# evergreen-ci/evergreen

Measured on NVIDIA H100. Metric: tasks scheduled/sec over N distros; host-allocator decisions/sec at 1/2/4/8 GPU, higher is better.
Workload: dtype int64

## Files before the change

### evergreen_b200/csrc/evg_plan_general.cuh

```cuda
#pragma once

#ifndef EVG_OCC_GLINK
#define EVG_OCC_GLINK 4
#endif
#ifndef EVG_OCC_GALLOC
#define EVG_OCC_GALLOC 4
#endif
#ifndef EVG_OCC_GFILL
#define EVG_OCC_GFILL 4
#endif
#ifndef EVG_OCC_GUNIT
#define EVG_OCC_GUNIT 4
#endif
#ifndef EVG_OCC_GBEST
#define EVG_OCC_GBEST 4
#endif
#ifndef EVG_GTASK_OCC
#define EVG_GTASK_OCC 2
#endif
constexpr int kGTile = 2048;

struct DGen {
  int64_t n_tiles;
  int64_t tile0;
// ... 65 lines not shown
}

__global__ void __launch_bounds__(256) k_gmark(DTasks T, DDistros D, DWork W, DGen G) {
  if (*W.err) return;
  const int tile = int(blockIdx.x + G.tile0);
  const int d = G.tile_distro[tile];
  const int64_t base = D.task_off[d], end = D.task_off[d + 1];
  const int64_t lo = max(G.tile_start[tile], base), hi = min(G.tile_start[tile] + kGTile, end);
  for (int64_t t = lo + threadIdx.x; t < hi; t += 256)
    for (int64_t e = T.dep_off[t]; e < T.dep_off[t + 1]; e++) W.has_dep[base + T.dep_idx[e]] = 1;
}

struct TileFold {
  unsigned int c[10];
  unsigned long long s[4];
  unsigned long long vmax, vmin;
};

__global__ void __launch_bounds__(256, EVG_GTASK_OCC) k_gtask(DTasks T, DDistros D, DWork W, DGen G, int64_t now, int any_complex) {
  if (*W.err) return;
  __shared__ TileFold F;
  __shared__ evg_distro_cfg s_cfg;
  __shared__ uint32_t s_nd[kNdTable];
  const int tile = int(blockIdx.x + G.tile0);
  const int d = G.tile_distro[tile];
  const int tid = threadIdx.x, lane = tid & 31;
  const unsigned full = 0xffffffffu;
  if (tid == 0) {
    for (int k = 0; k < 10; k++) F.c[k] = 0;
    for (int k = 0; k < 4; k++) F.s[k] = 0;
    F.vmax = 0ull; F.vmin = ~0ull;
    s_cfg = D.cfg[d];
  }
  __syncthreads();
  const evg_distro_cfg& cfg = s_cfg;
  const int64_t base = D.task_off[d], end = D.task_off[d + 1];
  const int64_t ts = G.tile_start[tile];
  const uint32_t ng = uint32_t(D.group_off[d + 1] - D.group_off[d]);
  const uint32_t ub = uint32_t(D.unit_base[d]);
  const bool gv = cfg.group_versions != 0;
  const int64_t threshold = cfg.target_time_ns;
  const PlannerFactors pf = clamp_factors(cfg);
  const Factors32 f32 = factors32(pf, now);
  const bool sane_clock = threshold >= 0 && now >= threshold;
  const int64_t wait_cutoff = wsub(now, threshold);
  const bool fast_clock = now >= 0 && pf.nd_int != 0;
  const bool incl = cfg.includes_dependencies != 0;
  if (tid < kNdTable) {
    const int64_t e = nd_table_entry(pf, tid);
    s_nd[tid] = (e >= 0 && e < int64_t(kNdTermLimit)) ? uint32_t(e) : 0xFFFFFFFFu;
  }
  __syncthreads();
  const bool dcomplex = any_complex && (ng > 0 || gv || (T.n_edges > 0 && T.dep_off[end] > T.dep_off[base]));

  unsigned int c_dm = 0, c_mq = 0, c_over = 0, c_wait = 0, c_sec = 0, c_ung = 0, c_ucnt = 0, c_uover = 0, c_uwait = 0, c_umq = 0;
  int64_t s_exp = 0, s_over = 0, s_uexp = 0, s_uover = 0;
  unsigned long long kmax = 0ull, kmin = ~0ull;

#pragma unroll 1
  for (int u = 0; u < 2; u++) {
    const int64_t t4 = ts + 4 * int64_t(u * 256 + tid);
    const bool live = t4 < end;
    int4 prio4 = make_int4(0, 0, 0, 0), nd4 = prio4, gid4 = make_int4(-1, -1, -1, -1), tgo4 = prio4, vid4 = prio4;
    uint4 fl4 = make_uint4(0, 0, 0, 0);
    uint32_t cmask = 0, womask = 0;
    if (live && dcomplex) {
      tgo4 = *reinterpret_cast<const int4*>(T.tgo + t4);
      if (gv) vid4 = *reinterpret_cast<const int4*>(T.vid + t4);
    }
    longlong2 ex01 = make_longlong2(0, 0), ex23 = ex01, qb01 = ex01, qb23 = ex01, wb01 = ex01, wb23 = ex01;
    if (live) {
      prio4 = *reinterpret_cast<const int4*>(T.priority + t4);
      nd4 = *reinterpret_cast<const int4*>(T.numdep + t4);
      gid4 = *reinterpret_cast<const int4*>(T.gid + t4);
      fl4 = *reinterpret_cast<const uint4*>(T.flags + t4);
      ex01 = *reinterpret_cast<const longlong2*>(T.expected + t4); ex23 = *reinterpret_cast<const longlong2*>(T.expected + t4 + 2);
      qb01 = *reinterpret_cast<const longlong2*>(T.qbasis + t4); qb23 = *reinterpret_cast<const longlong2*>(T.qbasis + t4 + 2);
      wb01 = *reinterpret_cast<const longlong2*>(T.wbasis + t4); wb23 = *reinterpret_cast<const longlong2*>(T.wbasis + t4 + 2);
    }
    int64_t doff[5] = {0, 0, 0, 0, 0};
    uint32_t hd4 = 0;
    if (live && dcomplex) {
      if (T.n_edges > 0) {
        const longlong2 d01 = *reinterpret_cast<const longlong2*>(T.dep_off + t4), d23 = *reinterpret_cast<const longlong2*>(T.dep_off + t4 + 2);
        doff[0] = d01.x; doff[1] = d01.y; doff[2] = d23.x; doff[3] = d23.y; doff[4] = T.dep_off[t4 + 4];
      }
      hd4 = *reinterpret_cast<const uint32_t*>(W.has_dep + t4);
    }
    const int32_t prio_[4] = {prio4.x, prio4.y, prio4.z, prio4.w}, nd_[4] = {nd4.x, nd4.y, nd4.z, nd4.w};
    const int32_t gid_[4] = {gid4.x, gid4.y, gid4.z, gid4.w};
    const uint32_t fl_[4] = {fl4.x, fl4.y, fl4.z, fl4.w};
    const int64_t ex_[4] = {ex01.x, ex01.y, ex23.x, ex23.y}, qb_[4] = {qb01.x, qb01.y, qb23.x, qb23.y};
    const int64_t wb_[4] = {wb01.x, wb01.y, wb23.x, wb23.y};
    int64_t vout[4];
    uint32_t eout[4], nd_term[4];
    bool wr_v[4], solo[4];
    bool dom = true;
#pragma unroll
    for (int m = 0; m < 4; m++) {
      const int64_t t = t4 + m;
      const bool valid = live & (t >= base) & (t < end);
      const int32_t prio = prio_[m], nd = nd_[m], gid = gid_[m];
      const uint32_t fl = fl_[m];
      const int64_t exp_ns = ex_[m], qb = qb_[m], wb = wb_[m];
      const bool dm = valid & ((fl & EVG_TF_DEPS_MET) != 0);
      const bool counted = valid & (!incl | dm);
      const bool over = counted & (exp_ns > threshold);
      const bool waited = sane_clock ? (wb < wait_cutoff) : (since(now, wb) > threshold);
      const bool wait_over = counted & dm & waited;
      const bool mq_dm = dm & ((fl & EVG_TF_REQ_MASK) == EVG_TF_REQ_MERGE_QUEUE);
      const bool ung = valid & (gid < 0);
      c_dm += dm; c_mq += mq_dm; c_over += over; c_wait += wait_over; c_sec += valid & ((fl & EVG_TF_OTHER_DISTRO) != 0);
      s_exp += counted ? exp_ns : 0;
      s_over += over ? exp_ns : 0;
      c_ung += ung; c_ucnt += ung & counted; c_uover += ung & over; c_uwait += ung & wait_over; c_umq += ung & mq_dm;
      s_uexp += (ung & counted) ? exp_ns : 0;
      s_uover += (ung & over) ? exp_ns : 0;
      const bool own_complex = valid & dcomplex & ((gid >= 0) | gv | (((hd4 >> (8 * m)) & 0xFFu) != 0));
      const bool complex_task = own_complex | (valid & dcomplex & (doff[m + 1] > doff[m]));
      const bool scores = valid & !own_complex;
      const uint32_t ndc = uint32_t(nd > 0 ? nd : 0);
      const uint32_t tab = s_nd[ndc < uint32_t(kNdTable) ? ndc : 0u];
      const uint32_t mul = (f32.ok & (ndc < kTask32Limit)) ? f32.nd * ndc : 0xFFFFFFFFu;
      nd_term[m] = ndc < uint32_t(kNdTable) ? tab : mul;
      dom = dom & (!scores | (score32_bad(now, prio, exp_ns, qb, nd_term[m]) == 0u));
      wr_v[m] = scores;
      solo[m] = scores & !complex_task;
      eout[m] = (valid & !complex_task) ? 1u : 0u;
      cmask |= (complex_task ? 1u : 0u) << m;
      womask |= (wait_over ? 1u : 0u) << m;
    }
    if (f32.ok_base && __all_sync(full, dom)) {
#pragma unroll
      for (int m = 0; m < 4; m++) vout[m] = int64_t(single_task_value32_nd(f32, now, prio_[m], ex_[m], qb_[m], nd_term[m], fl_[m]));
    } else {
#pragma unroll
      for (int m = 0; m < 4; m++) vout[m] = int64_t(score_slow(pf, fast_clock, wr_v[m], now, prio_[m], ex_[m], qb_[m], nd_[m], fl_[m]));
    }
#pragma unroll
    for (int m = 0; m < 4; m++) {
      const unsigned long long k = ord_i64(vout[m]);
      kmax = solo[m] ? max(kmax, k) : kmax;
      kmin = solo[m] ? min(kmin, k) : kmin;
    }
    if (!live) {
    } else if (t4 >= base && t4 + 3 < end) {
      *reinterpret_cast<longlong2*>(G.tv + t4) = make_longlong2(vout[0], vout[1]);
      *reinterpret_cast<longlong2*>(G.tv + t4 + 2) = make_longlong2(vout[2], vout[3]);
    } else {
#pragma unroll
      for (int m = 0; m < 4; m++)
        if (wr_v[m]) G.tv[t4 + m] = vout[m];
    }
    if (dcomplex && live) {
      if (t4 >= base && t4 + 3 < end) *reinterpret_cast<uint4*>(G.e + t4) = make_uint4(eout[0], eout[1], eout[2], eout[3]);
      else {
#pragma unroll
        for (int m = 0; m < 4; m++)
          if (t4 + m >= base && t4 + m < end) G.e[t4 + m] = eout[m];
      }
    }
    if (dcomplex) {
      __shared__ uint32_t s_wsum[8];
      __shared__ uint32_t s_lbase;
      const uint32_t mine = __popc(cmask);
      uint32_t inc = mine;
#pragma unroll
      for (int o = 1; o < 32; o <<= 1) { const uint32_t x = __shfl_up_sync(full, inc, o); if (lane >= o) inc += x; }
      if (lane == 31) s_wsum[tid >> 5] = inc;
      __syncthreads();
      uint32_t before = 0, total = 0;
#pragma unroll
      for (int w = 0; w < 8; w++) { const uint32_t x = s_wsum[w]; before += w < (tid >> 5) ? x : 0u; total += x; }
      if (total) {
        if (tid == 0) s_lbase = atomicAdd(G.ccount, total);
        __syncthreads();
        uint32_t pos = s_lbase + before + inc - mine;
        const int32_t vid_[4] = {vid4.x, vid4.y, vid4.z, vid4.w}, tgo_[4] = {tgo4.x, tgo4.y, tgo4.z, tgo4.w};
#pragma unroll
        for (int m = 0; m < 4; m++) {
          if (!((cmask >> m) & 1u)) continue;
          const uint32_t t = uint32_t(t4 + m), li = uint32_t(t4 + m - base);
          const int32_t gid = gid_[m], vid = vid_[m];
          const bool own_complex = (gid >= 0) | gv | (((hd4 >> (8 * m)) & 0xFFu) != 0);
          const uint32_t s_own = own_complex ? ub + own_slot_local(gid, vid, li, ng, gv) : kInactive;
          const uint32_t s_ver = (gid >= 0 && gv) ? ub + ng + uint32_t(vid) : kInactive;
          G.wl[pos] = make_uint4(t, uint32_t(d), s_own, s_ver);
          URec r;
          r.prio = prio_[m]; r.nd = nd_[m]; r.exp_ns = ex_[m]; r.qb = qb_[m]; r.tgo = tgo_[m];
          r.lif = li | (gid >= 0 ? kRecGrouped : 0u) | (((womask >> m) & 1u) ? kRecWaitOver : 0u) | ((fl_[m] & 0x3Fu) << 24);
          rec_store(G.pay + pos, r);
          pos++;
        }
      }
      __syncthreads();
    }
  }
  {
    unsigned int cs[10] = {c_dm, c_mq, c_over, c_wait, c_sec, c_ung, c_ucnt, c_uover, c_uwait, c_umq};
#pragma unroll
    for (int k = 0; k < 10; k++) cs[k] = __reduce_add_sync(full, cs[k]);
    int64_t ss[4] = {s_exp, s_over, s_uexp, s_uover};
#pragma unroll
    for (int k = 0; k < 4; k++) ss[k] = warp_sum64(ss[k]);
#pragma unroll
    for (int o = 16; o > 0; o >>= 1) {
      kmax = max(kmax, __shfl_xor_sync(full, kmax, o));
      kmin = min(kmin, __shfl_xor_sync(full, kmin, o));
    }
    if (lane == 0) {
#pragma unroll
      for (int k = 0; k < 10; k++) if (cs[k]) atomicAdd(&F.c[k], cs[k]);
#pragma unroll
      for (int k = 0; k < 4; k++) if (ss[k]) atomicAdd(&F.s[k], (unsigned long long)ss[k]);
      atomicMax(&F.vmax, kmax); atomicMin(&F.vmin, kmin);
    }
  }
  __syncthreads();
  if (tid < 16) {
    evg_queue_info* q = W.qinfo + d;
    switch (tid) {
      case 0: atomic_add64(&q->length_with_dependencies_met, F.c[0]); break;
      case 1: atomic_add64(&q->count_dep_filled_merge_queue_tasks, F.c[1]); break;
      case 2: atomic_add64(&q->count_duration_over_threshold, F.c[2]); break;
      case 3: atomic_add64(&q->count_wait_over_threshold, F.c[3]); break;
      case 4: atomic_add64(&q->secondary_queue, F.c[4]); break;
      case 5: atomic_add64(&q->has_ungrouped, F.c[5]); break;
      case 6: atomic_add64(&q->ungrouped.count, F.c[6]); break;
      case 7: atomic_add64(&q->ungrouped.count_duration_over_threshold, F.c[7]); break;
      case 8: atomic_add64(&q->ungrouped.count_wait_over_threshold, F.c[8]); break;
      case 9: atomic_add64(&q->ungrouped.count_dep_filled_merge_queue_tasks, F.c[9]); break;
      case 10: atomic_add64(&q->expected_duration, int64_t(F.s[0])); break;
      case 11: atomic_add64(&q->duration_over_threshold, int64_t(F.s[1])); break;
      case 12: atomic_add64(&q->ungrouped.expected_duration, int64_t(F.s[2])); break;
      case 13: atomic_add64(&q->ungrouped.duration_over_threshold, int64_t(F.s[3])); break;
      case 14: if (F.vmax > __ldcg(G.vmm + 2 * d)) atomicMax(G.vmm + 2 * d, F.vmax); break;
      case 15: if (F.vmin < __ldcg(G.vmm + 2 * d + 1)) atomicMin(G.vmm + 2 * d + 1, F.vmin); break;
    }
  }
}


struct WlTask {
  uint32_t t; int d; int64_t base; uint32_t li; bool own_complex; uint32_t s_own, s_ver;
};
__device__ __forceinline__ WlTask wl_task(const DDistros& D, const DGen& G, unsigned int k) {
  const uint4 e = G.wl[k];
  WlTask x;
  x.t = e.x; x.d = int(e.y); x.s_own = e.z; x.s_ver = e.w;
  x.base = D.task_off[x.d];
  x.li = uint32_t(int64_t(x.t) - x.base);
  x.own_complex = x.s_own != kInactive;
  return x;
}
template <typename F>
__device__ __forceinline__ void wl_pairs(const DTasks& T, const DGen& G, const WlTask& x, unsigned int k, F&& f) {
  if (x.own_complex) f(G.pown + k, x.s_own, true);
  if (x.s_ver != kInactive) f(G.pver + k, x.s_ver, false);
  if (T.n_edges > 0)
    for (int64_t e = T.dep_off[x.t]; e < T.dep_off[x.t + 1]; e++) {
      const uint32_t sl = G.sedge[e];
      if (sl != kInactive) f(G.pedge + e, sl, false);
    }
}

__global__ void __launch_bounds__(256, EVG_OCC_GLINK) k_glink(DTasks T, DDistros D, DWork W, DGen G, int64_t now) {
  if (*W.err) return;
  const unsigned int n = *G.ccount;
  for (unsigned int k = blockIdx.x * blockDim.x + threadIdx.x; k < n; k += gridDim.x * blockDim.x) {
    const WlTask x = wl_task(D, G, k);
    const uint32_t t = x.t;
    const int d = x.d;
    const uint32_t ub = uint32_t(D.unit_base[d]), ng = uint32_t(D.group_off[d + 1] - D.group_off[d]);
    if (x.own_complex && x.s_own - ub < ng) {
      const URec me = rec_load(G.pay + k);
      const evg_distro_cfg* cf = D.cfg + d;
      const uint32_t fl = (me.lif >> 24) & 0x3Fu;
      const int64_t exp_ns = me.exp_ns, threshold = cf->target_time_ns;
      const bool dm = (fl & EVG_TF_DEPS_MET) != 0;
      const bool counted = !cf->includes_dependencies || dm;
      const bool over = counted && exp_ns > threshold;
      const bool wait_over = (me.lif & kRecWaitOver) != 0;
      const bool mq_dm = dm && (fl & EVG_TF_REQ_MASK) == EVG_TF_REQ_MERGE_QUEUE;
      evg_group_info* g = W.ginfo + D.group_off[d] + (x.s_own - ub);
      atomic_add64(&g->count, counted);
      atomic_add64(&g->expected_duration, counted ? exp_ns : 0);
      atomic_add64(&g->count_duration_over_threshold, over);
      atomic_add64(&g->duration_over_threshold, over ? exp_ns : 0);
      atomic_add64(&g->count_wait_over_threshold, wait_over);
      atomic_add64(&g->count_dep_filled_merge_queue_tasks, mq_dm);
    }
    if (x.own_complex) G.pown[k] = atomicAdd(W.unit_n + x.s_own, 1u);
    if (x.s_ver != kInactive) G.pver[k] = atomicAdd(W.unit_n + x.s_ver, 1u);
    if (T.n_edges > 0) {
      const bool gv = D.cfg[d].group_versions != 0;
      const int64_t e0 = T.dep_off[t], e1 = T.dep_off[t + 1];
      for (int64_t e = e0; e < e1; e++) {
        const uint32_t dl = uint32_t(T.dep_idx[e]);
        const uint32_t sl = ub + own_slot_local(T.gid[x.base + dl], T.vid[x.base + dl], dl, ng, gv);
        bool dup = (sl == x.s_own) || (sl == x.s_ver);
        for (int64_t f = e0; f < e && !dup; f++) {
          const uint32_t fl2 = uint32_t(T.dep_idx[f]);
          dup = ub + own_slot_local(T.gid[x.base + fl2], T.vid[x.base + fl2], fl2, ng, gv) == sl;
        }
        G.sedge[e] = dup ? kInactive : sl;
        if (!dup) G.pedge[e] = atomicAdd(W.unit_n + sl, 1u);
      }
// ... 329 lines not shown
    } else {
#pragma unroll
      for (int m = 0; m < 8; m++) { const int64_t t = t8 + m; if (t >= base && t < end) G.e[t] = ps[m]; }
    }
    __syncthreads();
    const uint32_t total = s_total;
    const bool staged = total <= uint32_t(kStage);
#pragma unroll
    for (int m = 0; m < 8; m++) {
      const int64_t t = t8 + m;
      if (t >= base && t < end && !((dsp >> m) & 1u)) {
        if (staged) {
          const unsigned long long key = vmax_ord - ord_i64(vv[m]);
          const uint32_t q = ps[m] - p_tile;
          st_lo[q] = uint32_t(key); st_ix[q] = uint32_t(t - base);
          if (wide) st_hi[q] = uint32_t(key >> 32);
        } else {
          gen_put(G, base, ps[m], vmax_ord, wide, vv[m], uint32_t(t - base));
        }
      }
    }
    if (staged) {
      __syncthreads();
      uint32_t* dlo = G.key_lo[0] + base + p_tile;
      uint32_t* dix = G.idx[0] + base + p_tile;
      uint32_t* dhi = G.key_hi[0] + base + p_tile;
      for (uint32_t q = tid; q < total; q += 256) {
        dlo[q] = st_lo[q]; dix[q] = st_ix[q];
        if (wide) dhi[q] = st_hi[q];
      }
    }
  } else if (interior) {
    uint32_t kl[8], kh[8];
#pragma unroll
    for (int m = 0; m < 8; m++) {
      const unsigned long long key = vmax_ord - ord_i64(vv[m]);
      kl[m] = uint32_t(key); kh[m] = uint32_t(key >> 32);
    }
    const uint32_t p0 = uint32_t(t8 - base);
    *reinterpret_cast<uint4*>(G.key_lo[0] + t8) = make_uint4(kl[0], kl[1], kl[2], kl[3]);
    *reinterpret_cast<uint4*>(G.key_lo[0] + t8 + 4) = make_uint4(kl[4], kl[5], kl[6], kl[7]);
    *reinterpret_cast<uint4*>(G.idx[0] + t8) = make_uint4(p0, p0 + 1, p0 + 2, p0 + 3);
    *reinterpret_cast<uint4*>(G.idx[0] + t8 + 4) = make_uint4(p0 + 4, p0 + 5, p0 + 6, p0 + 7);
    if (wide) {
      *reinterpret_cast<uint4*>(G.key_hi[0] + t8) = make_uint4(kh[0], kh[1], kh[2], kh[3]);
      *reinterpret_cast<uint4*>(G.key_hi[0] + t8 + 4) = make_uint4(kh[4], kh[5], kh[6], kh[7]);
    }
  } else {
#pragma unroll
    for (int m = 0; m < 8; m++) {
      const int64_t t = t8 + m;
      if (t >= base && t < end) gen_put(G, base, uint32_t(t - base), vmax_ord, wide, vv[m], uint32_t(t - base));
    }
  }
}

__global__ void __launch_bounds__(256) k_gplace_disp(DTasks T, DDistros D, DWork W, DGen G) {
  const unsigned int n = *G.ccount;
  for (unsigned int k = blockIdx.x * blockDim.x + threadIdx.x; k < n; k += gridDim.x * blockDim.x) {
  const uint4 ent = G.wl[k];
  const uint32_t t = ent.x;
  if (!(W.has_dep[t] & 2)) continue;
  const int d = int(ent.y);
  const int64_t base = D.task_off[d];
  const uint4 tie = G.tie[k];
  const uint32_t a = tie.x, myrk = tie.y, slot = tie.z;
  uint32_t pos = G.e[base + a];
  const uint32_t cnt = W.unit_n[slot];
  if (cnt <= 64) {
    pos += __popcll(W.unit_mask[slot] & ((1ull << myrk) - 1ull));
  } else {
    const uint32_t* run = G.run + W.head[slot];
    for (uint32_t i = 0; i < cnt; i++) {
      const uint4 tq = G.tie[run[i] & kRunEntry];
      if (tq.z == slot && tq.y < myrk) pos++;
    }
  }
  gen_put(G, base, pos, G.vmm[2 * d], gen_bits(G, d) > 32, G.tv[t], uint32_t(int64_t(t) - base));
  }
}

__device__ __forceinline__ bool gen_tile(const DDistros& D, const DGen& G, int tile, int j, int* d_out, int64_t* seg, int64_t* lo,
                                         int* cnt, bool* wide) {
  const int d = G.tile_distro[tile];
  const int bits = gen_bits(G, d);
  if (j >= gen_npass(bits)) return false;
  const int64_t base = D.task_off[d], end = D.task_off[d + 1];
  const int64_t a = max(G.tile_start[tile], base), b = min(G.tile_start[tile] + kGTile, end);
  *d_out = d; *seg = base; *lo = a; *cnt = int(b - a); *wide = bits > 32;
  return true;
}

__global__ void __launch_bounds__(256) k_ghist(int j, DDistros D, DGen G) {
  if (j >= *G.maxpass) return;
  int d, cnt; int64_t seg, lo; bool wide;
  const int tile = int(blockIdx.x + G.tile0);
  if (!gen_tile(D, G, tile, j, &d, &seg, &lo, &cnt, &wide)) return;
  const uint32_t* src = (j < 4 ? G.key_lo[j & 1] : G.key_hi[j & 1]) + lo;
  const int shift = 8 * (j & 3);
  __shared__ uint32_t h[256];
  h[threadIdx.x] = 0;
  __syncthreads();
  for (int i = threadIdx.x; i < cnt; i += 256) atomicAdd(&h[(src[i] >> shift) & 255u], 1u);
  __syncthreads();
  G.tile_hist[int64_t(tile) * 256 + threadIdx.x] = h[threadIdx.x];
}

__global__ void __launch_bounds__(1024) k_gdscan(int j, const int32_t* __restrict__ general_list, DGen G) {
  if (j >= *G.maxpass) return;
  const int d = general_list[blockIdx.x];
  if (j >= gen_npass(gen_bits(G, d))) return;
  const int dg = threadIdx.x & 255, grp = threadIdx.x >> 8;
  const int64_t t0 = G.dtile_off[d], nt = G.dtile_off[d + 1] - t0;
  const int64_t per = (nt + 3) / 4;
  const int64_t a = t0 + (grp * per < nt ? grp * per : nt), b = t0 + ((grp + 1) * per < nt ? (grp + 1) * per : nt);
  uint32_t* h = G.tile_hist + dg;
  uint32_t sum = 0;
  int64_t tile = a;
  for (; tile + 8 <= b; tile += 8) {
    uint32_t x[8];
#pragma unroll
    for (int k = 0; k < 8; k++) x[k] = h[(tile + k) * 256];
#pragma unroll
    for (int k = 0; k < 8; k++) sum += x[k];
  }
  for (; tile < b; tile++) sum += h[tile * 256];
  __shared__ uint32_t part[4][256];
  __shared__ uint32_t s[256];
  part[grp][dg] = sum;
  __syncthreads();
  const uint32_t total = part[0][dg] + part[1][dg] + part[2][dg] + part[3][dg];
  if (grp == 0) s[dg] = total;
  __syncthreads();
  for (int o = 1; o < 256; o <<= 1) {
    uint32_t v = 0;
    if (grp == 0 && dg >= o) v = s[dg - o];
    __syncthreads();
    if (grp == 0) s[dg] += v;
    __syncthreads();
  }
  uint32_t run = s[dg] - total;
  for (int g = 0; g < grp; g++) run += part[g][dg];
  tile = a;
  for (; tile + 8 <= b; tile += 8) {
    uint32_t x[8];
#pragma unroll
    for (int k = 0; k < 8; k++) x[k] = h[(tile + k) * 256];
#pragma unroll
    for (int k = 0; k < 8; k++) { h[(tile + k) * 256] = run; run += x[k]; }
  }
  for (; tile < b; tile++) { const uint32_t x = h[tile * 256]; h[tile * 256] = run; run += x; }
}

template <bool WIDE>
__device__ __forceinline__ void gscatter_tile(int j, const DGen& G, int tile, int64_t seg, int64_t lo, int cnt, uint32_t (*wcnt)[256],
                                              uint32_t* s_lo, uint32_t* s_ix, uint32_t* s_hi, int32_t* s_delta, uint32_t* s_wsum) {
  constexpr bool wide = WIDE;
  const int sb = j & 1, db = sb ^ 1;
  const int tid = threadIdx.x, warp = tid >> 5, lane = tid & 31;
#pragma unroll
  for (int w = 0; w < 8; w++) wcnt[w][tid] = 0u;
  __syncthreads();
  const unsigned lt = (1u << lane) - 1u;
  const int shift = 8 * (j & 3);
  const bool use_hi = j >= 4;
  const uint32_t* src_lo = G.key_lo[sb] + lo;
  const uint32_t* src_hi = G.key_hi[sb] + lo;
  const uint32_t* src_ix = G.idx[sb] + lo;
  uint32_t kl[8], kh[8], ix[8], dg[8], rk[8];
#pragma unroll
  for (int k = 0; k < 8; k++) {
    const int i = (warp * 8 + k) * 32 + lane;
    const bool ok = i < cnt;
    kl[k] = ok ? src_lo[i] : 0u;
    kh[k] = (ok && wide) ? src_hi[i] : 0u;
    ix[k] = ok ? src_ix[i] : 0u;
  }
  unsigned peers[8];
#pragma unroll
  for (int k = 0; k < 8; k++) {
    const int i = (warp * 8 + k) * 32 + lane;
    dg[k] = i < cnt ? (((use_hi ? kh[k] : kl[k]) >> shift) & 255u) : 256u;
    peers[k] = __match_any_sync(0xffffffffu, dg[k]);
  }
#pragma unroll
  for (int k = 0; k < 8; k++) {
    rk[k] = 0;
    if (dg[k] < 256u && (peers[k] & lt) == 0u) rk[k] = atomicAdd(&wcnt[warp][dg[k]], uint32_t(__popc(peers[k])));
  }
#pragma unroll
  for (int k = 0; k < 8; k++) rk[k] = __shfl_sync(0xffffffffu, rk[k], __ffs(peers[k]) - 1) + uint32_t(__popc(peers[k] & lt));
  __syncthreads();
  {
    uint32_t x[8], tot = 0;
#pragma unroll
    for (int w = 0; w < 8; w++) { x[w] = wcnt[w][tid]; tot += x[w]; }
    uint32_t inc = tot;
#pragma unroll
    for (int o = 1; o < 32; o <<= 1) { const uint32_t y = __shfl_up_sync(0xffffffffu, inc, o); if (lane >= o) inc += y; }
    if (lane == 31) s_wsum[warp] = inc;
    __syncthreads();
    uint32_t before = 0;
#pragma unroll
    for (int w = 0; w < 8; w++) before += w < warp ? s_wsum[w] : 0u;
    const uint32_t lbase = before + inc - tot;
    s_delta[tid] = int32_t(G.tile_hist[int64_t(tile) * 256 + tid]) - int32_t(lbase);
    uint32_t run = lbase;
#pragma unroll
    for (int w = 0; w < 8; w++) { wcnt[w][tid] = run; run += x[w]; }
  }
  __syncthreads();
#pragma unroll
  for (int k = 0; k < 8; k++) {
    if (dg[k] < 256u) {
      const uint32_t lp = wcnt[warp][dg[k]] + rk[k];
      s_lo[lp] = kl[k];
      s_ix[lp] = ix[k];
      if (wide) s_hi[lp] = kh[k];
    }
  }
  __syncthreads();
  uint32_t* dst_lo = G.key_lo[db] + seg;
  uint32_t* dst_hi = G.key_hi[db] + seg;
  uint32_t* dst_ix = G.idx[db] + seg;
  for (int i = tid; i < cnt; i += 256) {
    const uint32_t a = s_lo[i], h = wide ? s_hi[i] : 0u;
    const uint32_t dgt = ((use_hi ? h : a) >> shift) & 255u;
    const int64_t pos = int64_t(s_delta[dgt]) + i;
    dst_lo[pos] = a;
    dst_ix[pos] = s_ix[i];
    if (wide) dst_hi[pos] = h;
  }
}

__global__ void __launch_bounds__(256, 4) k_gscatter(int j, DDistros D, DGen G) {
  if (j >= *G.maxpass) return;
  int d, cnt; int64_t seg, lo; bool wide;
  const int tile = int(blockIdx.x + G.tile0);
  if (!gen_tile(D, G, tile, j, &d, &seg, &lo, &cnt, &wide)) return;
  __shared__ uint32_t wcnt[8][256];
  __shared__ uint32_t s_lo[kGTile], s_ix[kGTile], s_hi[kGTile];
  __shared__ int32_t s_delta[256];
  __shared__ uint32_t s_wsum[8];
  if (wide) gscatter_tile<true>(j, G, tile, seg, lo, cnt, wcnt, s_lo, s_ix, s_hi, s_delta, s_wsum);
  else gscatter_tile<false>(j, G, tile, seg, lo, cnt, wcnt, s_lo, s_ix, s_hi, s_delta, s_wsum);
}

__global__ void __launch_bounds__(256) k_gemit(DDistros D, DGen G, int32_t* __restrict__ order, int64_t* __restrict__ total_value) {
  const int tile = int(blockIdx.x + G.tile0);
  const int d = G.tile_distro[tile];
  const int64_t base = D.task_off[d], end = D.task_off[d + 1];
  const int64_t lo = max(G.tile_start[tile], base), hi = min(G.tile_start[tile] + kGTile, end);
  const int bits = gen_bits(G, d);
  const int fin = gen_npass(bits) & 1;
  const bool wide = bits > 32;
  const unsigned long long vmax_ord = G.vmm[2 * d];
  for (int64_t p = lo + threadIdx.x; p < hi; p += 256) {
    unsigned long long key = G.key_lo[fin][p];
    if (wide) key |= (unsigned long long)G.key_hi[fin][p] << 32;
    order[p] = int32_t(G.idx[fin][p]);
    total_value[p] = unord_i64(vmax_ord - key);
  }
}
```

### evergreen_b200/csrc/evg_sched.cu

```cuda
#include <cuda_runtime.h>
#include <stdarg.h>
#include <stdint.h>
#include <stdio.h>
#include <string.h>

#include <algorithm>
#include <type_traits>
#include <cstdlib>
#include <future>
#include <mutex>
#include <string>
#include <vector>

#include "evg_score.cuh"
#include "evg_intern.h"

using namespace evg;

namespace {

thread_local std::string g_err;

int fail(int code, const char* fmt, ...) {
  char buf[512];
// ... 1423 lines not shown
  w.best_pair = c->b_bestpair.as<uint32_t>();
  w.buf[0].key_v = c->b_kv.as<uint64_t>();
  w.qinfo = c->b_qinfo.as<evg_queue_info>(); w.ginfo = c->b_ginfo.as<evg_group_info>();
  return w;
}
DGen dgen(const evg_ctx* c) {
  DGen g;
  g.n_tiles = c->NT;
  g.tile0 = 0;
  g.tile_distro = c->b_tiledistro.as<int32_t>(); g.tile_start = c->b_tilestart.as<int64_t>();
  g.dtile_off = c->b_dtileoff.as<int64_t>();
  g.vmm = c->b_vmm.as<unsigned long long>();
  for (int k = 0; k < 2; k++) {
    g.key_lo[k] = c->b_klo[k].as<uint32_t>(); g.key_hi[k] = c->b_khi[k].as<uint32_t>(); g.idx[k] = c->b_ix[k].as<uint32_t>();
  }
  g.e = c->b_e.as<uint32_t>(); g.tile_sum = c->b_tilesum.as<uint32_t>(); g.tile_hist = c->b_tilehist.as<uint32_t>();
  g.wl = c->b_wl.as<uint4>();
  g.pay = c->b_pay.as<URec>();
  g.pown = c->b_place.as<uint32_t>();
  g.pver = c->b_place.as<uint32_t>() + (c->Tgc + 1);
  g.pedge = c->b_eplace.as<uint32_t>();
  g.sedge = c->b_eplace.as<uint32_t>() + (c->E + 1);
  g.ccount = c->b_gmisc.as<unsigned int>();
  g.maxpass = c->b_gmisc.as<int32_t>() + 1;
  g.rcount = c->b_gmisc.as<unsigned int>() + 2;
  g.hcount = c->b_gmisc.as<unsigned int>() + 3;
  g.bcount = c->b_gmisc.as<unsigned int>() + 4;
  g.blist = c->b_blist.as<uint2>();
  g.rank = c->b_rank.as<uint32_t>();
  g.hlist = c->b_hlist.as<uint2>();
  g.usum = c->b_usum.as<uint4>();
  g.run = c->b_run.as<uint32_t>();
  g.tie = c->b_tie.as<uint4>();
  g.tv = c->b_tv.as<int64_t>();
  return g;
}

#define LOCK(c) std::lock_guard<std::recursive_mutex> lock_((c)->mu)
#define LAUNCH_ON(c, st, kernel, grid, block, ...)                           \
  do {                                                                       \
    if ((grid) > 0) {                                                        \
      kernel<<<(grid), (block), 0, (st)>>>(__VA_ARGS__);                     \
      (c)->launches++;                                                       \
    }                                                                        \
  } while (0)
#define LAUNCH(c, kernel, grid, block, ...) LAUNCH_ON(c, (c)->stream, kernel, grid, block, __VA_ARGS__)

int run_alloc_range(evg_ctx* c, int64_t now, int32_t d0, int32_t d1) {
  DHosts h;
  h.n = c->H; h.flags = c->b_hflags.as<uint32_t>(); h.gid = c->b_hgid.as<int32_t>();
  h.expected = c->b_hexp.as<int64_t>(); h.stddev = c->b_hstd.as<int64_t>(); h.start = c->b_hstart.as<int64_t>();
  h.host_off = c->b_hostoff.as<int64_t>(); h.cfg = c->b_acfg.as<evg_alloc_cfg>();
  if (c->ext_result && c->ext_capacity < c->Dn) return fail(EVG_ERR_INVALID, "bound result buffer holds %lld rows, need %d", (long long)c->ext_capacity, c->Dn);
  CK(c->b_gs.ensure(sizeof(GroupScratch) * size_t(c->G + 1)));
  const int split = (d1 - d0) >= 4096 ? 1 : 0;
  const bool listed = split && c->alist_valid && d0 == 0 && d1 == c->Dn;
  const int32_t* al = listed ? c->b_alist.as<int32_t>() : nullptr;
  const int64_t teams = listed ? c->n_alist : int64_t(d1 - d0);
  if (c->max_groups > kWideAllocGroups)
    LAUNCH(c, k_alloc<128>, unsigned(teams), 128, h, d0, d1, c->b_groupoff.as<int64_t>(), c->b_qinfo.as<evg_queue_info>(),
           c->b_ginfo.as<evg_group_info>(), c->b_gs.as<GroupScratch>(), now, c->result_ptr(), c->b_status.as<int32_t>(), split, al, int32_t(c->n_alist));
  else
    LAUNCH(c, k_alloc<32>, grid_for(teams, 4), 128, h, d0, d1, c->b_groupoff.as<int64_t>(), c->b_qinfo.as<evg_queue_info>(),
           c->b_ginfo.as<evg_group_info>(), c->b_gs.as<GroupScratch>(), now, c->result_ptr(), c->b_status.as<int32_t>(), split, al, int32_t(c->n_alist));
  if (split)
    LAUNCH(c, k_alloc_groupless, grid_for(d1 - d0, 128), 128, h, d0, d1, c->b_groupoff.as<int64_t>(), c->b_qinfo.as<evg_queue_info>(), now,
           c->result_ptr(), c->b_status.as<int32_t>());
  CK(cudaGetLastError());
  return EVG_OK;
}
int run_alloc(evg_ctx* c, int64_t now) { return run_alloc_range(c, now, 0, c->Dn); }

template <int THREADS, int ITEMS, int MIN_CTAS>
int launch_smem(evg_ctx* c, cudaStream_t st, const DTasks& dt, const DDistros& dd, const DWork& w, const int32_t* list, int32_t n,
                int64_t now, int lists_needed = 0, const int32_t* list_count = nullptr) {
  if (n <= 0) return EVG_OK;
  const size_t bytes = PlanSmem<THREADS, ITEMS>::kBytes;
  CK(cudaFuncSetAttribute(k_plan_smem<THREADS, ITEMS, MIN_CTAS>, cudaFuncAttributeMaxDynamicSharedMemorySize, int(bytes)));
  k_plan_smem<THREADS, ITEMS, MIN_CTAS><<<unsigned(n), THREADS, bytes, st>>>(dt, dd, w, list, list_count, now, lists_needed,
                                                                          c->b_order.as<int32_t>(), c->b_tv.as<int64_t>());
  c->launches++;
  return EVG_OK;
}

template <int THREADS, int CAP, int OCC>
int launch_cta(evg_ctx* c, cudaStream_t st, const DTasks& dt, const DDistros& dd, const DWork& w, const int32_t* list, int32_t n,
               int64_t now, int32_t* punt_list, int32_t* punt_count) {
  if (n <= 0) return EVG_OK;
  const size_t bytes = PlanCta<THREADS, CAP>::kBytes;
  CK(cudaFuncSetAttribute(k_plan_cta<THREADS, CAP, OCC>, cudaFuncAttributeMaxDynamicSharedMemorySize, int(bytes)));
  k_plan_cta<THREADS, CAP, OCC><<<unsigned(n), THREADS, bytes, st>>>(dt, dd, w, list, now, c->t_pad, c->b_order.as<int32_t>(),
                                                                  c->b_tv.as<int64_t>(), punt_list, punt_count);
  c->launches++;
  return EVG_OK;
}

int launch_tiny(evg_ctx* c, cudaStream_t st, const DTasks& dt, const DDistros& dd, const DWork& w, const int32_t* list, int32_t n,
                int64_t now, int lists_needed) {
  if (n <= 0) return EVG_OK;
  if (lists_needed) return launch_smem<128, 8, 8>(c, st, dt, dd, w, list, n, now, 1);
  k_plan_warp<<<grid_for(int64_t(n) * 32, 256), 256, 0, st>>>(dt, dd, w, list, n, now, c->b_order.as<int32_t>(), c->b_tv.as<int64_t>());
  c->launches++;
  return EVG_OK;
}

int prepare_general(evg_ctx* c, cudaStream_t s, int32_t d0, int32_t d1) {
  const int64_t t0 = c->h_taskoff[d0], t1 = c->h_taskoff[d1], u0 = c->h_unitbase[d0], u1 = c->h_unitbase[d1];
  const int64_t g0 = c->h_groupoff[d0], g1 = c->h_groupoff[d1], e0 = c->h_edgeoff[d0], e1 = c->h_edgeoff[d1];
  CK(cudaMemsetAsync(c->b_qinfo.as<evg_queue_info>() + d0, 0, sizeof(evg_queue_info) * size_t(d1 - d0), s));
  if (g1 > g0) CK(cudaMemsetAsync(c->b_ginfo.as<evg_group_info>() + g0, 0, sizeof(evg_group_info) * size_t(g1 - g0), s));
  if (c->general_complex) {
    const size_t nt = size_t(t1 - t0);
    CK(cudaMemsetAsync(c->b_hasdep.as<uint8_t>() + t0, 0, nt, s));
    CK(cudaMemsetAsync(c->b_unitn.as<uint32_t>() + u0, 0, sizeof(uint32_t) * size_t(u1 - u0), s));
  }
  return EVG_OK;
}

int run_general(evg_ctx* c, cudaStream_t st, const DTasks& dt, const DDistros& dd, const DWork& w, int64_t now, int32_t gfirst,
                int32_t gcount) {
  if (gcount <= 0) return EVG_OK;
  DGen g = dgen(c);
  const int gc = c->general_complex;
  const std::vector<int32_t>& gh = c->routes[kGeneral].h;
  const int32_t d_first = gh[size_t(gfirst)], d_last = gh[size_t(gfirst + gcount - 1)];
  g.tile0 = c->h_dtileoff[size_t(d_first)];
  const unsigned nt = unsigned(c->h_dtileoff[size_t(d_last) + 1] - g.tile0);
  const int32_t* gl = c->routes[kGeneral].b.as<int32_t>() + gfirst;
  LAUNCH_ON(c, st, k_ginit, grid_for(gcount, 256), 256, g, gl, gcount);
  if (gc && c->E > 0) LAUNCH_ON(c, st, k_gmark, nt, 256, dt, dd, w, g);
  if (c->timed) CK(cudaEventRecord(c->ev_gt0, st));
  LAUNCH_ON(c, st, k_gtask, nt, 256, dt, dd, w, g, now, gc);
  if (c->timed) { CK(cudaEventRecord(c->ev_gt1, st)); c->general_timed = true; }
  const unsigned wl_grid = unsigned(std::min<int64_t>(std::max<int64_t>(1, (c->Tgc + 255) / 256), int64_t(c->num_sms) * 16));
  if (gc) {
    LAUNCH_ON(c, st, k_glink, wl_grid, 256, dt, dd, w, g, now);
    LAUNCH_ON(c, st, k_galloc, wl_grid, 256, dt, dd, w, g);
    LAUNCH_ON(c, st, k_gfill, wl_grid, 256, dt, dd, w, g);
    LAUNCH_ON(c, st, k_gunit, wl_grid, 256, dd, w, g, now);
    LAUNCH_ON(c, st, k_grank, wl_grid, 256, w, g);
    LAUNCH_ON(c, st, k_gbest, wl_grid, 256, dt, dd, w, g, c->bd_valid ? 1 : 0);
  }
  LAUNCH_ON(c, st, k_gsched, grid_for(gcount, 128), 128, g, gl, gcount);
  if (gc) {
    LAUNCH_ON(c, st, k_gsum, nt, 256, dd, g);
    LAUNCH_ON(c, st, k_gscan, unsigned(gcount), 1024, g, gl);
  }
  LAUNCH_ON(c, st, k_gplace, nt, 256, dd, w, g, gc);
  if (gc) LAUNCH_ON(c, st, k_gplace_disp, wl_grid, 256, dt, dd, w, g);
  if (c->timed) CK(cudaEventRecord(c->ev_sort0, st));
  for (int j = 0; j < 8; j++) {
    LAUNCH_ON(c, st, k_ghist, nt, 256, j, dd, g);
    LAUNCH_ON(c, st, k_gdscan, unsigned(gcount), 1024, j, gl, g);
    LAUNCH_ON(c, st, k_gscatter, nt, 256, j, dd, g);
  }
  if (c->timed) CK(cudaEventRecord(c->ev_sort1, st));
  LAUNCH_ON(c, st, k_gemit, nt, 256, dd, g, c->b_order.as<int32_t>(), c->b_tv.as<int64_t>());
  const int64_t g0 = c->h_groupoff[size_t(d_first)], g1 = c->h_groupoff[size_t(d_last) + 1];
  LAUNCH_ON(c, st, k_finalize_info, grid_for(std::max<int64_t>(d_last + 1 - d_first, g1 - g0), 256), 256, dd, w, d_first, d_last + 1, g0, g1);
  return EVG_OK;
}

int ensure_aux_streams(evg_ctx* c) {
  if (c->ev_fork) return EVG_OK;
  for (int k = 0; k < evg_ctx::kAux; k++) {
    CK(cudaStreamCreateWithFlags(&c->s_aux[k], cudaStreamNonBlocking));
    CK(cudaEventCreateWithFlags(&c->ev_join[k], cudaEventDisableTiming));
  }
  CK(cudaEventCreateWithFlags(&c->ev_fork, cudaEventDisableTiming));
  return EVG_OK;
}

enum class Mode { kResident, kBreakdown, kPipelined };

int plan_route(evg_ctx* c, int r, Mode mode, cudaStream_t st, const DTasks& dt, const DDistros& dd, const DWork& w, int64_t now,
               int32_t first, int32_t n, int32_t* punt, int32_t* punt_count) {
  if (n <= 0) return EVG_OK;
  const int bd = mode == Mode::kBreakdown ? 1 : 0;
  const int32_t* list = punt;
  if (r != kPunted) list = (mode != Mode::kPipelined && largest_first(r) ? c->routes[r].lpt : c->routes[r].b).as<int32_t>() + first;
  if (bd && is_cta(r)) return launch_smem<EVG_C_THREADS, EVG_C_ITEMS, 1>(c, st, dt, dd, w, list, n, now, 1);
  int rc;
  switch (r) {
    case kCtaC: return launch_cta<kNT_C, kNCapC, kNOccC>(c, st, dt, dd, w, list, n, now, punt, punt_count);
    case kCtaB: return launch_cta<kNT_B, kNCapB, kNOccB>(c, st, dt, dd, w, list, n, now, punt, punt_count);
    case kCtaA:
      if (mode == Mode::kResident) {
        if ((rc = launch_cta<kNT_A, kNCapA, kNOccA>(c, st, dt, dd, w, list, c->nNA_big, now, punt, punt_count)) != EVG_OK) return rc;
        return launch_cta<kNT_S, kNCapS, kNOccS>(c, st, dt, dd, w, list + c->nNA_big, n - c->nNA_big, now, punt, punt_count);
      }
      return launch_cta<kNT_A, kNCapA, kNOccA>(c, st, dt, dd, w, list, n, now, punt, punt_count);
    case kPunted:
      if (mode == Mode::kResident && c->max_cta_tasks <= kCapA) return launch_smem<128, 8, 8>(c, st, dt, dd, w, list, n, now, 0, punt_count);
      if (mode == Mode::kResident && c->max_cta_tasks <= kCapB) return launch_smem<256, 16, 3>(c, st, dt, dd, w, list, n, now, 0, punt_count);
      return launch_smem<EVG_C_THREADS, EVG_C_ITEMS, 1>(c, st, dt, dd, w, list, n, now, 0, punt_count);
    case kSmemC: return launch_smem<EVG_C_THREADS, EVG_C_ITEMS, 1>(c, st, dt, dd, w, list, n, now, bd);
    case kSmemB: return launch_smem<256, 16, 3>(c, st, dt, dd, w, list, n, now, bd);
    case kSmemA: return launch_smem<128, 8, 8>(c, st, dt, dd, w, list, n, now, bd);
    case kWarp: return launch_tiny(c, st, dt, dd, w, list, n, now, bd);
    default: {
      const std::vector<int32_t>& gh = c->routes[kGeneral].h;
      if (mode == Mode::kPipelined && (rc = prepare_general(c, st, gh[size_t(first)], gh[size_t(first + n - 1)] + 1)) != EVG_OK) return rc;
      return run_general(c, st, dt, dd, w, now, first, n);
    }
  }
}

int run_plan(evg_ctx* c, int64_t now, uint32_t opts) {
  const int64_t T = c->T;
  const int32_t D = c->Dn;
  cudaStream_t s = c->stream;
  DTasks dt = dtasks(c);
  DDistros dd = ddistros(c);
  DWork w = dwork(c);
  int64_t* bd = nullptr;
  c->bd_valid = false;
  if (opts & EVG_OPT_BREAKDOWN) {
    CK(c->b_bd.ensure(sizeof(int64_t) * EVG_BD_N * size_t(T + 1)));
    bd = c->b_bd.as<int64_t>();
    c->bd_valid = true;
  }
  c->sort_slot = -1;
  if (D == 0) {
    if (c->timed) { CK(cudaEventRecord(c->ev_sort0, s)); CK(cudaEventRecord(c->ev_sort1, s)); }
    return EVG_OK;
  }
  const std::vector<int32_t>& gh = c->routes[kGeneral].h;
  const bool general = !gh.empty();
  if (bd && c->any_complex) CK(cudaMemsetAsync(c->b_bestpair.p, 0xFF, sizeof(uint32_t) * size_t(T + 1), s));
  const int32_t n_new = bd ? 0 : c->routes[kCtaA].n() + c->routes[kCtaB].n() + c->routes[kCtaC].n();
  if (n_new > 0) CK(cudaMemsetAsync(c->b_puntcnt.p, 0, sizeof(int32_t), s));
  if (general) { int rcg = prepare_general(c, s, gh.front(), gh.back() + 1); if (rcg != EVG_OK) return rcg; }
  bool busy[evg_ctx::kAux] = {};
  for (int r = 0; r < kRoutes; r++) busy[kRouteStream[r]] |= c->routes[r].n() > 0;
  const bool fork = std::count(busy, busy + evg_ctx::kAux, true) > 1;
  if (fork) {
    int rc0 = ensure_aux_streams(c);
    if (rc0 != EVG_OK) return rc0;
    CK(cudaEventRecord(c->ev_fork, s));
    for (int k = 0; k < evg_ctx::kAux; k++) CK(cudaStreamWaitEvent(c->s_aux[k], c->ev_fork, 0));
  }
  int rc;
  const int slot = int(c->runs % evg_ctx::kRing);
  const Mode mode = bd ? Mode::kBreakdown : Mode::kResident;
  for (int r : {kCtaC, kCtaB, kCtaA, kPunted, kSmemC, kSmemB, kSmemA, kWarp, kGeneral}) {
    const int32_t n = r == kPunted ? n_new : c->routes[r].n();
    cudaStream_t sr = fork ? c->s_aux[kRouteStream[r]] : s;
    const bool time_it = c->timed && !general && c->sort_slot < 0 && n > 0 && (r == kSmemC || (r == kCtaC && !bd));
    if (time_it) CK(cudaEventRecord(c->ring0[slot], sr));
    if ((rc = plan_route(c, r, mode, sr, dt, dd, w, now, 0, n, c->b_punt.as<int32_t>(), c->b_puntcnt.as<int32_t>())) != EVG_OK) return rc;
    if (time_it) { CK(cudaEventRecord(c->ring1[slot], sr)); c->runs++; c->sort_slot = slot; }
  }
  if (fork) {
    for (int k = 0; k < evg_ctx::kAux; k++) {
      CK(cudaEventRecord(c->ev_join[k], c->s_aux[k]));
      CK(cudaStreamWaitEvent(s, c->ev_join[k], 0));
    }
  }
  if (bd) LAUNCH(c, k_breakdown, grid_for(T, 256), 256, dt, dd, w, c->b_run.as<uint32_t>(), c->b_pay.as<URec>(), now, c->any_complex, c->b_order.as<int32_t>(), bd);
  CK(cudaGetLastError());
  return EVG_OK;
}

}

extern "C" {

const char* evg_last_error(void) { return g_err.c_str(); }
int evg_abi_version(void) { return EVG_ABI_VERSION; }

int evg_init(int device, void* stream, evg_ctx** out) {
  if (!out) return fail(EVG_ERR_INVALID, "evg_init: out is null");
  *out = nullptr;
  int n = 0;
  cudaError_t e = cudaGetDeviceCount(&n);
  if (e != cudaSuccess || n == 0) return fail(EVG_ERR_CUDA, "no CUDA device: %s (libevgsched has no CPU fallback)", cudaGetErrorString(e));
  if (device < 0 || device >= n) return fail(EVG_ERR_INVALID, "device %d out of range (%d devices)", device, n);
  CK(cudaSetDevice(device));
  cudaDeviceProp prop;
  CK(cudaGetDeviceProperties(&prop, device));
  if (prop.major != 9 || prop.minor != 0)
    return fail(EVG_ERR_CUDA, "device %d is sm_%d%d; this library is built for sm_90a only", device, prop.major, prop.minor);
  evg_ctx* c = new evg_ctx();
  c->device = device;
  c->num_sms = prop.multiProcessorCount;
  if (stream) { c->stream = reinterpret_cast<cudaStream_t>(stream); c->own_stream = false; }
  else { CK(cudaStreamCreateWithFlags(&c->stream, cudaStreamNonBlocking)); c->own_stream = true; }
  CK(cudaEventCreate(&c->ev_begin)); CK(cudaEventCreate(&c->ev_sort0));
  CK(cudaEventCreate(&c->ev_sort1)); CK(cudaEventCreate(&c->ev_end));
  CK(cudaEventCreate(&c->ev_gt0)); CK(cudaEventCreate(&c->ev_gt1));
  for (int k = 0; k < evg_ctx::kRing; k++) { CK(cudaEventCreate(&c->ring0[k])); CK(cudaEventCreate(&c->ring1[k])); }
  *out = c;
  return EVG_OK;
}

void evg_shutdown(evg_ctx* c) {
  if (!c) return;
  cudaSetDevice(c->device);
  cudaStreamSynchronize(c->stream);
  for (int k = 0; k < evg_ctx::kRing; k++) { if (c->ring0[k]) cudaEventDestroy(c->ring0[k]); if (c->ring1[k]) cudaEventDestroy(c->ring1[k]); }
  cudaEventDestroy(c->ev_begin); cudaEventDestroy(c->ev_sort0); cudaEventDestroy(c->ev_sort1); cudaEventDestroy(c->ev_end);
  cudaEventDestroy(c->ev_gt0); cudaEventDestroy(c->ev_gt1);
  for (int k = 0; k < evg_ctx::kMaxChunks; k++) { if (c->ev_h[k]) cudaEventDestroy(c->ev_h[k]); if (c->ev_c[k]) cudaEventDestroy(c->ev_c[k]); }
  if (c->s_h2d) cudaStreamDestroy(c->s_h2d);
  if (c->s_d2h) cudaStreamDestroy(c->s_d2h);
  for (int k = 0; k < evg_ctx::kAux; k++) { if (c->s_aux[k]) cudaStreamDestroy(c->s_aux[k]); if (c->ev_join[k]) cudaEventDestroy(c->ev_join[k]); }
  if (c->ev_fork) cudaEventDestroy(c->ev_fork);
// ... 2154 lines not shown
```

Before: 4.418 billion.

## Fuse final radix-sort scatter with emit and replace match_any with ballots

On the last radix pass, the scatter kernel writes the order and total_value outputs directly instead of writing keys back to global memory for a separate emit kernel. The emit kernel now only handles distros with zero key bits. The per-digit warp peer mask now comes from nine ballots instead of __match_any_sync. A score-write condition also changes from dcomplex to any_complex. Together these drop one global round trip over the sorted keys, in exchange for extra ballot instructions and some risk around the changed condition and the final-pass detection.

```diff
diff --git a/evergreen_b200/csrc/evg_plan_general.cuh b/evergreen_b200/csrc/evg_plan_general.cuh
--- a/evergreen_b200/csrc/evg_plan_general.cuh
+++ b/evergreen_b200/csrc/evg_plan_general.cuh
@@ -241,7 +241,7 @@
       for (int m = 0; m < 4; m++)
         if (wr_v[m]) G.tv[t4 + m] = vout[m];
     }
-    if (dcomplex && live) {
+    if (any_complex && live) {
       if (t4 >= base && t4 + 3 < end) *reinterpret_cast<uint4*>(G.e + t4) = make_uint4(eout[0], eout[1], eout[2], eout[3]);
       else {
 #pragma unroll
@@ -877,9 +877,21 @@
   for (; tile < b; tile++) { const uint32_t x = h[tile * 256]; h[tile * 256] = run; run += x; }
 }
 
+__device__ __forceinline__ unsigned digit_peers(uint32_t dg) {
+  unsigned m = 0xffffffffu;
+#pragma unroll
+  for (int b = 0; b < 9; b++) {
+    const unsigned x = __ballot_sync(0xffffffffu, (dg >> b) & 1u);
+    m &= ((dg >> b) & 1u) ? x : ~x;
+  }
+  return m;
+}
+
 template <bool WIDE>
 __device__ __forceinline__ void gscatter_tile(int j, const DGen& G, int tile, int64_t seg, int64_t lo, int cnt, uint32_t (*wcnt)[256],
-                                              uint32_t* s_lo, uint32_t* s_ix, uint32_t* s_hi, int32_t* s_delta, uint32_t* s_wsum) {
+                                              uint32_t* s_lo, uint32_t* s_ix, uint32_t* s_hi, int32_t* s_delta, uint32_t* s_wsum,
+                                              bool last, unsigned long long vmax_ord, int32_t* __restrict__ order,
+                                              int64_t* __restrict__ total_value) {
   constexpr bool wide = WIDE;
   const int sb = j & 1, db = sb ^ 1;
   const int tid = threadIdx.x, warp = tid >> 5, lane = tid & 31;
@@ -906,7 +918,7 @@
   for (int k = 0; k < 8; k++) {
     const int i = (warp * 8 + k) * 32 + lane;
     dg[k] = i < cnt ? (((use_hi ? kh[k] : kl[k]) >> shift) & 255u) : 256u;
-    peers[k] = __match_any_sync(0xffffffffu, dg[k]);
+    peers[k] = digit_peers(dg[k]);
   }
 #pragma unroll
   for (int k = 0; k < 8; k++) {
@@ -945,6 +957,18 @@
     }
   }
   __syncthreads();
+  if (last) {
+    int32_t* dst_o = order + seg;
+    int64_t* dst_v = total_value + seg;
+    for (int i = tid; i < cnt; i += 256) {
+      const uint32_t a = s_lo[i], h = wide ? s_hi[i] : 0u;
+      const uint32_t dgt = ((use_hi ? h : a) >> shift) & 255u;
+      const int64_t pos = int64_t(s_delta[dgt]) + i;
+      dst_o[pos] = int32_t(s_ix[i]);
+      dst_v[pos] = unord_i64(vmax_ord - ((unsigned long long)h << 32 | a));
+    }
+    return;
+  }
   uint32_t* dst_lo = G.key_lo[db] + seg;
   uint32_t* dst_hi = G.key_hi[db] + seg;
   uint32_t* dst_ix = G.idx[db] + seg;
@@ -958,32 +982,31 @@
   }
 }
 
-__global__ void __launch_bounds__(256, 4) k_gscatter(int j, DDistros D, DGen G) {
+__global__ void __launch_bounds__(256, 4) k_gscatter(int j, DDistros D, DGen G, int32_t* __restrict__ order,
+                                                     int64_t* __restrict__ total_value) {
   if (j >= *G.maxpass) return;
   int d, cnt; int64_t seg, lo; bool wide;
   const int tile = int(blockIdx.x + G.tile0);
   if (!gen_tile(D, G, tile, j, &d, &seg, &lo, &cnt, &wide)) return;
+  const bool last = j == gen_npass(gen_bits(G, d)) - 1;
+  const unsigned long long vmax_ord = G.vmm[2 * d];
   __shared__ uint32_t wcnt[8][256];
   __shared__ uint32_t s_lo[kGTile], s_ix[kGTile], s_hi[kGTile];
   __shared__ int32_t s_delta[256];
   __shared__ uint32_t s_wsum[8];
-  if (wide) gscatter_tile<true>(j, G, tile, seg, lo, cnt, wcnt, s_lo, s_ix, s_hi, s_delta, s_wsum);
-  else gscatter_tile<false>(j, G, tile, seg, lo, cnt, wcnt, s_lo, s_ix, s_hi, s_delta, s_wsum);
+  if (wide) gscatter_tile<true>(j, G, tile, seg, lo, cnt, wcnt, s_lo, s_ix, s_hi, s_delta, s_wsum, last, vmax_ord, order, total_value);
+  else gscatter_tile<false>(j, G, tile, seg, lo, cnt, wcnt, s_lo, s_ix, s_hi, s_delta, s_wsum, last, vmax_ord, order, total_value);
 }
 
 __global__ void __launch_bounds__(256) k_gemit(DDistros D, DGen G, int32_t* __restrict__ order, int64_t* __restrict__ total_value) {
   const int tile = int(blockIdx.x + G.tile0);
   const int d = G.tile_distro[tile];
+  if (gen_bits(G, d) != 0) return;
   const int64_t base = D.task_off[d], end = D.task_off[d + 1];
   const int64_t lo = max(G.tile_start[tile], base), hi = min(G.tile_start[tile] + kGTile, end);
-  const int bits = gen_bits(G, d);
-  const int fin = gen_npass(bits) & 1;
-  const bool wide = bits > 32;
   const unsigned long long vmax_ord = G.vmm[2 * d];
   for (int64_t p = lo + threadIdx.x; p < hi; p += 256) {
-    unsigned long long key = G.key_lo[fin][p];
-    if (wide) key |= (unsigned long long)G.key_hi[fin][p] << 32;
-    order[p] = int32_t(G.idx[fin][p]);
-    total_value[p] = unord_i64(vmax_ord - key);
-  }
-}
+    order[p] = int32_t(G.idx[0][p]);
+    total_value[p] = unord_i64(vmax_ord - G.key_lo[0][p]);
+  }
+}
diff --git a/evergreen_b200/csrc/evg_sched.cu b/evergreen_b200/csrc/evg_sched.cu
--- a/evergreen_b200/csrc/evg_sched.cu
+++ b/evergreen_b200/csrc/evg_sched.cu
@@ -1599,7 +1599,7 @@
   for (int j = 0; j < 8; j++) {
     LAUNCH_ON(c, st, k_ghist, nt, 256, j, dd, g);
     LAUNCH_ON(c, st, k_gdscan, unsigned(gcount), 1024, j, gl, g);
-    LAUNCH_ON(c, st, k_gscatter, nt, 256, j, dd, g);
+    LAUNCH_ON(c, st, k_gscatter, nt, 256, j, dd, g, c->b_order.as<int32_t>(), c->b_tv.as<int64_t>());
   }
   if (c->timed) CK(cudaEventRecord(c->ev_sort1, st));
   LAUNCH_ON(c, st, k_gemit, nt, 256, dd, g, c->b_order.as<int32_t>(), c->b_tv.as<int64_t>());
```

Measured after the change: 4.538 billion, median of 6. +2.7%, better.
